# samanseifi/pyRMT

Measured on AMD Instinct MI355X. Metric: cell-updates/s (full RMT step) at N=4096; achieved HBM GB/s vs peak, higher is better.
Workload: dtype f64; 1 GPU; soft_disc_in_lid_driven N=4096 semilagrangian (configs 2/4 loop body); grid=4096, parallelism=single-gpu

## Files before the change

### pyrmt_amd/csrc/extrap.hip

```cpp
#include "extrap.hpp"
#include <cstring>
#include "exp_glibc.h"

namespace rmt {

constexpr int EXW = 8;
constexpr int EX_RING = 1024;
constexpr int EX_WIN = 81;
constexpr unsigned EX_DONE = 0x7fffffffu;
constexpr long EX_SPIN_LIMIT = 1L << 25;

__global__ void __launch_bounds__(256) k_ex_bits(const double *__restrict__ phi, int ny, int nx,
                                                 int W, int ML, u64 *__restrict__ kbits,
                                                 u64 *__restrict__ K,
                                                 unsigned char *__restrict__ rowcand,
                                                 int *__restrict__ jrange,
                                                 const double *__restrict__ X1,
                                                 const double *__restrict__ X2,
                                                 double *__restrict__ X1o,
                                                 double *__restrict__ X2o, int copy,
                                                 const u64 *__restrict__ kin) {
    const int j = blockIdx.y, i = blockIdx.x * 256 + threadIdx.x;
    const long c = (long)j * nx + i;
    const bool in = i < nx;
// ... 607 lines not shown
    const int ML = std::max(max_layers, 1), W = (nx + 63) / 64;
    const long plane = (long)ny * W;
    const long interior = (long)std::max(ny - 2, 0) * std::max(nx - 2, 0);
    const long maxt = std::max(64L, std::min((long)ML * interior, 4L * ML * (nx + ny) + 4096));
    char *p = (char *)base;
    size_t o = 0;
    auto take = [&](size_t n) { char *q = p ? p + o : nullptr; o += (n + 255) & ~(size_t)255; return q; };
    ExWs w{};
    w.kbits = (u64 *)take(plane * 8);
    w.cbits = (u64 *)take(plane * 8);
    w.Kold = (u64 *)take(plane * 8 * ML);
    w.rowcand = (unsigned char *)take(ny);
    w.jrange = (int *)take(64);
    w.status = w.jrange + 2;
    w.T = (u64 *)take(plane * 8 * ML);
    w.ACC = (u64 *)take(plane * 8 * ML);
    w.KN = (u64 *)take(plane * 8 * ML);
    w.rowcnt = (int *)take((size_t)ML * ny * 4);
    w.rowoff = (int *)take((size_t)ML * (ny + 1) * 4);
    w.wordoff = (int *)take(plane * 4 * ML);
    w.cbase = (int *)take((size_t)ML * ny * 4);
    w.tcell = (long long *)take(maxt * 8);
    w.recoff = (long long *)take(maxt * 8);
    w.rec_by_chain = (long long *)take(maxt * 8);
    w.chain_of = (int *)take(maxt * 4);
    w.dmark = (int *)take(maxt * 4);
    w.part = (unsigned char *)take(maxt);
    w.loc = (int *)take(maxt * 4);
    w.inv = (int *)take(maxt * 4);
    w.wnext = (int *)take(maxt * 4);
    w.gval = (double *)take(maxt * 16);
    w.rej = (int *)take((size_t)ML * EX_MAXREJ * 4);
    w.ctl = (int *)take(EXC_WORDS * 4);
    const long long cap = (1LL << 31) - 65536;
    w.slots = !bump && maxt * (long long)CH_MAXREC <= cap;
    w.arena_bytes = w.slots ? maxt * (long long)CH_MAXREC : std::min(maxt * 2560LL, cap);
    w.arena = take(w.arena_bytes);
    w.maxt = maxt;
    w.plane = plane;
    w.maxseg = maxt / PX_K + EX_MAXL + 2;
    if (px) {
        w.pns = (int *)take(maxt * 4);
        w.pnd = (int *)take(maxt * 4);
        w.pkey = (int *)take(maxt * PX_S * 4);
        w.pbeta = (double *)take(maxt * PX_S * 8);
        w.pval = (double2 *)take(maxt * 16);
        w.pc = (double2 *)take(maxt * 16);
        w.live = (unsigned char *)take(maxt);
        w.shdr = (int *)take(w.maxseg * PX_H * 4);
        w.sF = (int *)take(w.maxseg * PX_F * 4);
        w.sMT = (double *)take(w.maxseg * PX_F * PX_K * 8);
        w.sNT = (double *)take(w.maxseg * PX_K * PX_K * 8);
        w.sd = (double2 *)take(w.maxseg * PX_K * 16);
        w.spk = (double *)take(w.maxseg * PX_PB * 8);
    }
    if (bytes) *bytes = o;
    return w;
}

int extrap_none_rows(rmt_ctx *ctx, const u64 *kbits, int ny, int nx, double dx, double dy,
                     int jb, int je, int *ctl) {
    const double r = 4 * std::sqrt(dx * dx + dy * dy);
    if (je > jb)
        k_ex_none<<<grid1d(je - jb, 4), 256, 0, ctx->stream>>>(kbits, ny, nx, (nx + 63) / 64, dx,
                                                               dy, r * r, ctl, jb, je);
    RMT_LAUNCHED();
    return RMT_OK;
}

size_t extrap_workspace(int ny, int nx, int max_layers, bool px) {
    size_t b = 0;
    extrap_layout(nullptr, ny, nx, max_layers, &b, px);
    return b;
}

int extrap_geometry(rmt_ctx *ctx, const double *X1, const double *X2, const double *phi,
                    double dx, double dy, int max_layers, double *X1o, double *X2o,
                    const u64 *kin, const ExtrapCall &call) {
    const int ny = ctx->ny, nx = ctx->nx;
    const int W = (nx + 63) / 64;
    RMT_CHECK(max_layers > 0 && ny >= 3 && nx >= 3 && ny < (1 << 20) && nx < (1 << 30),
              RMT_EINVAL, "extrapolation grid size");
    const int force = g_ex_mode;
    const bool chain = force != 1 && extrap_chain_supported(ny, nx, max_layers);
    const bool par = chain && force == 0 && extrap_par_enabled();
    RMT_TRY(ensure_bytes(ctx, extrap_workspace(ny, nx, max_layers, par)));
    const ExWs ws = extrap_layout(ctx->bytes, ny, nx, max_layers, nullptr, par,
                                  ctx->opt.ex_arena_bump);
    ctx->ex_layers = max_layers;
    ctx->ex_chain = chain;
    ctx->ex_par = par;
    const int copy = (X1o != X1) || (X2o != X2);
    if (kin && !copy)
        k_ex_bits_w<<<grid1d((long)ny * W, 256), 256, 0, ctx->stream>>>(
            kin, ny, W, max_layers, ws.kbits, ws.Kold, ws.rowcand, ws.jrange);
    else
        k_ex_bits<<<dim3((nx + 255) / 256, ny), 256, 0, ctx->stream>>>(
            phi, ny, nx, W, max_layers, ws.kbits, ws.Kold, ws.rowcand, ws.jrange, X1, X2, X1o,
            X2o, copy, kin);
    RMT_HIP(hipMemsetAsync(ws.status, 0, 4 * sizeof(int), ctx->stream));
    if (chain) {
        RMT_HIP(hipMemsetAsync(ws.ctl, 0, EXC_WORDS * sizeof(int), ctx->stream));
        if (force == 2) {
            const int one = 1;
            RMT_HIP(hipMemcpyAsync(ws.ctl + EXC_FALLBACK, &one, sizeof(int),
                                   hipMemcpyHostToDevice, ctx->stream));
        }
        const double r = 4 * std::sqrt(dx * dx + dy * dy);
        int jb = 0, je = ny;
        if (call.none_rows[1] > call.none_rows[0]) {
            jb = std::max(0, call.none_rows[0]);
            je = std::min(ny, call.none_rows[1]);
        }
        if (call.none_wide && call.cand && je > jb) {
            int *cnt = call.cand + call.cand_cap;
            RMT_HIP(hipMemsetAsync(cnt, 0, sizeof(int), ctx->stream));
            int wb = 0, we = W;
            if (call.none_cols[1] > call.none_cols[0]) {
                wb = std::max(0, call.none_cols[0]);
                we = std::min(W, call.none_cols[1]);
            }
            k_ex_cand<<<grid1d((long)(je - jb) * (we - wb), 256), 256, 0, ctx->stream>>>(
                ws.kbits, ny, nx, W, jb, je, wb, we, call.cand, call.cand_cap, cnt);
            k_ex_none_list<<<1024, 256, 0, ctx->stream>>>(ws.kbits, ny, nx, W, dx, dy, r * r,
                                                           ws.ctl, jb, je, call.cand,
                                                           call.cand_cap, cnt);
        } else {
            k_ex_none<<<call.none_wide ? grid1d(std::max(je - jb, 1), 4)
                                          : std::min<unsigned>(grid1d(ny, 4), 64),
                        256, 0, ctx->stream>>>(
                ws.kbits, ny, nx, W, dx, dy, r * r, ws.ctl, jb, je);
        }
        k_ex_none_fin<<<1, 1, 0, ctx->stream>>>(ws.ctl);
        RMT_LAUNCHED();
        if (call.none_host && force == 0) {
            int any = 1;
            RMT_HIP(hipMemcpyAsync(&any, ws.ctl + EXC_ANY, sizeof(int), hipMemcpyDeviceToHost,
                                   ctx->stream));
            RMT_HIP(hipStreamSynchronize(ctx->stream));
            if (!any) { ctx->ex_noop_skip = true; return RMT_OK; }
        }
        if (par) {
            RMT_TRY(extrap_chain_prep_px(ctx, ws, dx, dy, max_layers));
            RMT_TRY(extrap_par_geometry(ctx, ws, dx, dy, max_layers));
        } else {
            RMT_TRY(extrap_chain_prep(ctx, ws, X1o, X2o, dx, dy, max_layers));
        }
    }
    const int *ctl = chain ? ws.ctl : nullptr;
    k_ex_dilate<<<grid1d((long)ny * W, 256), 256, 0, ctx->stream>>>(
        ws.kbits, ny, nx, W, max_layers, ws.cbits, ws.rowcand, ws.jrange, ctl);
    RMT_LAUNCHED();
    return RMT_OK;
}

int extrap_finish(rmt_ctx *ctx, double dx, double dy, int max_layers, double *X1o, double *X2o,
                  int *dev_status, const ExtrapCall &call) {
    const int ny = ctx->ny, nx = ctx->nx;
    const int W = (nx + 63) / 64;
    const bool par = ctx->ex_par;
    const ExWs ws = extrap_layout(ctx->bytes, ny, nx, max_layers, nullptr, par,
                                  ctx->opt.ex_arena_bump);
    const int force = g_ex_mode;
    if (ctx->ex_noop_skip) {
        ctx->ex_noop_skip = false;
        if (dev_status) RMT_HIP(hipMemsetAsync(dev_status, 0, 2 * sizeof(int), ctx->stream));
        if (call.chain_event) RMT_HIP(hipEventRecord(call.chain_event, ctx->stream));
        return RMT_OK;
    }
    const bool chain = ctx->ex_chain && !par;
    const int *ctl = ctx->ex_chain ? ws.ctl : nullptr;
    if (chain) RMT_TRY(extrap_chain_values(ctx, ws, X1o, X2o, dx, dy, max_layers, call));
    if (ctx->prof && !chain && !par) RMT_HIP(hipEventRecord(ctx->ev[2], ctx->stream));
    ExSweep A{X1o, X2o, ws.kbits, ws.cbits, ws.Kold, ws.rowcand, ws.jrange, ny, nx, W,
              max_layers, dx, dy, ws.status, ctl};
    const bool prof = ctx->opt.ex_profile != 0;
    const bool defer = chain && call.sweep_deferred && call.chain_event;
    RMT_CHECK(!defer || !dev_status, RMT_EINVAL,
              "extrap_finish: a deferred sweep leaves the status to the caller");
    if (defer) {
    } else if (!prof) {
        k_ex_sweep<false><<<1, EXW * 64, 0, ctx->stream>>>(A, nullptr);
        RMT_LAUNCHED();
    } else {
        long long *gp = nullptr, hp[EX_NPROF];
        int hs[2];
        RMT_HIP(hipMalloc(&gp, sizeof(hp)));
        RMT_HIP(hipMemsetAsync(gp, 0, sizeof(hp), ctx->stream));
        hipEvent_t e0, e1;
        RMT_HIP(hipEventCreate(&e0)); RMT_HIP(hipEventCreate(&e1));
        RMT_HIP(hipEventRecord(e0, ctx->stream));
        k_ex_sweep<true><<<1, EXW * 64, 0, ctx->stream>>>(A, gp);
        RMT_LAUNCHED();
        RMT_HIP(hipEventRecord(e1, ctx->stream));
        RMT_HIP(hipMemcpyAsync(hp, gp, sizeof(hp), hipMemcpyDeviceToHost, ctx->stream));
        RMT_HIP(hipMemcpyAsync(hs, ws.status, sizeof(hs), hipMemcpyDeviceToHost, ctx->stream));
        RMT_HIP(hipStreamSynchronize(ctx->stream));
        float ms = 0;
        RMT_HIP(hipEventElapsedTime(&ms, e0, e1));
        fprintf(stderr, "[ex-prof] %.3f ms fitted=%d rows=%lld | ticket+targets %.3g rowwait %.3g "
                "window %.3g wait %.3g load %.3g sum %.3g solve+store %.3g (Mclk, all waves)\n",
                ms, hs[0], hp[7], hp[0] / 1e6, hp[6] / 1e6, hp[1] / 1e6, hp[2] / 1e6,
                hp[3] / 1e6, hp[4] / 1e6, hp[5] / 1e6);
        (void)hipEventDestroy(e0); (void)hipEventDestroy(e1); (void)hipFree(gp);
    }
// ... 124 lines not shown
```

### pyrmt_amd/csrc/extrap.hpp

```cpp
#pragma once
#include "rmt_internal.hpp"

namespace rmt {

typedef unsigned long long u64;

constexpr int EX_MAXL = 8;
constexpr int CH_R = 2048;
#ifndef RMT_CH_W
#define RMT_CH_W 16
#endif
constexpr int CH_W = RMT_CH_W;
constexpr int CH_HDR = 24;
constexpr int CH_TVS = 88;
constexpr int CH_MAXREC = 8 * (CH_HDR + 6 * CH_TVS + 4 * 64);
constexpr int EX_MAXREJ = 4096;
constexpr int EX_DCAP = 8192;

constexpr int CH_MAXP = 8;
enum { EXC_FALLBACK = 0, EXC_ABORT = 1, EXC_FILLED = 2, EXC_ARENA = 4, EXC_REJ = 8,
       EXC_BASE = 8 + EX_MAXL, EXC_ANY = 8 + 2 * EX_MAXL, EXC_NOOP = EXC_ANY + 1,
       EXC_CMIN = EXC_ANY + 2, EXC_CMAX = EXC_ANY + 3, EXC_NPART = EXC_ANY + 4,
       EXC_WSTART = EXC_NPART + CH_MAXP + 1,
       EXC_NCOL = EXC_WSTART + CH_MAXP * CH_W,
       EXC_NLG = EXC_NCOL + 1,
       EXC_WORDS = EXC_NLG + 8 };
constexpr unsigned long long CH_GSENT = 0x7ff00000000bad01ull;
enum { EXA_CHAIN = 1, EXA_RELINK = 7, EXA_SWEEP = 8, EXA_PAR = 9 };
constexpr int EXA_TAG = 1 << 30;
__device__ __forceinline__ int exa_code(int kind, int part, int id) {
    return EXA_TAG | (kind << 26) | ((part & 15) << 22) | (id < 0 ? 0x3fffff : min(id, 0x3fffff));
}
__device__ __forceinline__ void exa_report(int *status, int code) {
    atomicCAS(status + 1, 0, code);
}
constexpr int PX_K = 64;
constexpr int PX_F = 64;
constexpr int PX_S = 81;
constexpr int PX_H = 8;
constexpr int PX_PB = 768;

struct ExWs {
    u64 *kbits, *cbits, *Kold;
    unsigned char *rowcand;
    int *jrange, *status;
    u64 *T, *ACC, *KN;
    int *rowcnt, *rowoff, *wordoff, *cbase;
    long long *tcell, *recoff, *rec_by_chain;
    int *chain_of, *dmark;
    unsigned char *part;
    int *loc, *inv;
    int *wnext;
    double *gval;
    int *rej;
    int *ctl;
    int *pns, *pnd;
    int *pkey;
    double *pbeta;
    double2 *pval, *pc;
    unsigned char *live;
    int *shdr, *sF;
    double *sMT, *sNT;
    double2 *sd;
    double *spk;
    long maxseg;
    char *arena;
    long long arena_bytes;
    int slots;
    long maxt;
    long plane;
};

ExWs extrap_layout(void *base, int ny, int nx, int max_layers, size_t *bytes, bool px = false,
                   bool bump = false);
int extrap_chain_prep(rmt_ctx *ctx, const ExWs &ws, const double *X1o, const double *X2o,
                      double dx, double dy, int ML);
int extrap_chain_values(rmt_ctx *ctx, const ExWs &ws, const double *X1o, const double *X2o,
                        double dx, double dy, int ML, const ExtrapCall &call = {});
int extrap_chain_run(rmt_ctx *ctx, const ExWs &ws, const double *X1o, const double *X2o, int ML,
                     const ExtrapCall &call = {});
bool extrap_chain_supported(int ny, int nx, int ML);
int extrap_chain_prep_px(rmt_ctx *ctx, const ExWs &ws, double dx, double dy, int ML);
int extrap_par_geometry(rmt_ctx *ctx, const ExWs &ws, double dx, double dy, int ML);
int extrap_par_values(rmt_ctx *ctx, const ExWs &ws, double *X1o, double *X2o, int ML);

}
```

### pyrmt_amd/csrc/extrap_chain.hip

```cpp
#include "extrap.hpp"
#include "exp_glibc.h"
#include <algorithm>
#include <cstdio>
#include <cstdlib>
#include <vector>

namespace rmt {

constexpr int EXS = 82;
constexpr long long CH_CRIT = 1LL << 16;

__device__ __forceinline__ u64 ld_l2(const u64 *p) {
    return __hip_atomic_load(p, __ATOMIC_RELAXED, __HIP_MEMORY_SCOPE_AGENT);
}
__device__ __forceinline__ int wave_incl_scan(int v, int lane) {
#pragma unroll
    for (int d = 1; d < 64; d <<= 1) {
        const int t = __shfl_up(v, d);
        if (lane >= d) v += t;
    }
    return v;
}
__device__ __forceinline__ u64 rl64(u64 v, int l) {
    const unsigned lo = __builtin_amdgcn_readlane((unsigned)v, l);
    const unsigned hi = __builtin_amdgcn_readlane((unsigned)(v >> 32), l);
    return ((u64)hi << 32) | lo;
}
__device__ __forceinline__ double rlf(double v, int l) {
    return __longlong_as_double((long long)rl64((u64)__double_as_longlong(v), l));
}
__device__ __forceinline__ int ex_id(const ExWs &ws, int ny, int Ls, int jj, long o, u64 bit) {
    return ws.ctl[EXC_BASE + Ls] + ws.rowoff[(long)Ls * (ny + 1) + jj] +
           ws.wordoff[(long)Ls * ws.plane + o] + __popcll(ws.T[(long)Ls * ws.plane + o] & (bit - 1));
}

__global__ void __launch_bounds__(256) k_tg_rows(ExWs ws, int ny, int nx, int W, int L) {
    const int lane = threadIdx.x & 63, j = blockIdx.x * 4 + (threadIdx.x >> 6);
    if (j >= ny) return;
    const long plane = ws.plane;
    const u64 *Kpp = L >= 2 ? ws.KN + (long)(L - 2) * plane : ws.kbits;
    const u64 *Ap = L >= 1 ? ws.ACC + (long)(L - 1) * plane : nullptr;
    auto K = [&](int jj, int w) -> u64 {
        if (jj < 0 || jj >= ny || w < 0 || w >= W) return 0;
// ... 138 lines not shown
    __builtin_amdgcn_fence(__ATOMIC_SEQ_CST, "wavefront");
    double acc = 0.0;
    if (lane < 6) {
        const double2 *t2 = (const double2 *)(tb + lane * EXS);
        double2 t[40];
#pragma unroll
        for (int q2 = 0; q2 < 40; ++q2) t[q2] = t2[q2];
        const double last = tb[lane * EXS + 80];
#pragma unroll
        for (int q2 = 0; q2 < 40; ++q2) { acc += t[q2].x; acc += t[q2].y; }
        acc += last;
    }
    __builtin_amdgcn_wave_barrier();
    __builtin_amdgcn_fence(__ATOMIC_SEQ_CST, "wavefront");
    const double A00 = rlf(acc, 0), A01 = rlf(acc, 1), A02 = rlf(acc, 2);
    const double A11 = rlf(acc, 3), A12 = rlf(acc, 4), A22 = rlf(acc, 5);
    const double M[9] = {A00, A01, A02, A01, A11, A12, A02, A12, A22};
    const double det = (M[0] * (M[4] * M[8] - M[5] * M[7])
                      - M[1] * (M[3] * M[8] - M[5] * M[6])
                      + M[2] * (M[3] * M[7] - M[4] * M[6]));
    const bool accept = count >= 3 && fabs(det) > 1e-10;
    if (!accept) {
        if (lane == 0) ws.recoff[id] = -1;
        return false;
    }
    if (A.norec) return true;
    const u64 lt = (1ull << lane) - 1;
    const u64 tl = il & ~((qf >= 64) ? ~0ull : ((1ull << qf) - 1));
    const u64 th = ih & ~((qf >= 64) ? ((1ull << (qf - 64)) - 1) : 0ull);
    const int n = __popcll(tl) + __popcll(th), npad = (n + 7) & ~7;
    const int nd = __popcll(dl) + __popcll(dh);
    const long long bytes = ((8LL * (CH_HDR + 4 * nd + 6 * npad)) + 63) & ~63LL;
    unsigned long long off = 0;
    if (nd > 64) {
        if (lane == 0) { ws.ctl[EXC_FALLBACK] = 1; ws.recoff[id] = -1; }
        return true;
    }
    if (ws.slots) {
        off = (unsigned long long)id * CH_MAXREC;
    } else {
        if (lane == 0) {
            off = atomicAdd((unsigned long long *)(ws.ctl + EXC_ARENA), (unsigned long long)bytes);
            if ((long long)(off + bytes) > ws.arena_bytes) ws.ctl[EXC_FALLBACK] = 1;
        }
        off = rl64(off, 0);
    }
    if ((long long)(off + bytes) > ws.arena_bytes) {
        if (lane == 0) ws.recoff[id] = -1;
        return true;
    }
    double *rec = (double *)(ws.arena + off);
    double *dyn = rec + CH_HDR;
    double *tv = dyn + 4 * nd;
#pragma unroll
    for (int h = 0; h < 2; ++h) {
        const bool term = h ? ((th >> lane) & 1) && lane < 17 : (tl >> lane) & 1;
        if (!term) continue;
        const int k = h ? __popcll(tl) + __popcll(th & lt) : __popcll(tl & lt);
        const double wa0 = w[h] * 1.0, wa1 = w[h] * xi[h], wa2 = w[h] * yi[h];
        if (!st[h]) {
            const int dk = h ? __popcll(dl) + __popcll(dh & lt) : __popcll(dl & lt);
            dyn[4 * dk] = __longlong_as_double(((long long)src[h] << 32) | (unsigned)k);
            dyn[4 * dk + 1] = wa0; dyn[4 * dk + 2] = wa1; dyn[4 * dk + 3] = wa2;
        }
    }
    if (lane < 6 * (npad - n)) tv[(lane / (npad - n)) * npad + n + lane % (npad - n)] = 0.0;
    if (lane == 0) {
// ... 107 lines not shown
            const double2 *t2 = (const double2 *)(T + lane * EXS);
            double2 t[40];
#pragma unroll
            for (int q2 = 0; q2 < 40; ++q2) t[q2] = t2[q2];
            const double last = T[lane * EXS + 80];
#pragma unroll
            for (int q2 = 0; q2 < 40; ++q2) { acc += t[q2].x; acc += t[q2].y; }
            acc += last;
        }
        __builtin_amdgcn_wave_barrier();
        __builtin_amdgcn_fence(__ATOMIC_SEQ_CST, "wavefront");
        double *rec = (double *)(ws.arena + ((r & 0xffffffffLL) << 6));
        const long long meta = __double_as_longlong(rec[1]);
        const int npad = (int)(meta & 0xffffffff), nd = (int)((meta >> 32) & 0x7fffffff);
        double *tv = rec + CH_HDR + 4 * nd;
        const u64 il = __ballot(inc[0]), ih = __ballot(inc[1] && lane < 17);
        const u64 lt = (1ull << lane) - 1;
        const u64 tl = il & ~((qf >= 64) ? ~0ull : ((1ull << qf) - 1));
        const u64 th = ih & ~((qf >= 64) ? ((1ull << (qf - 64)) - 1) : 0ull);
#pragma unroll
        for (int h = 0; h < 2; ++h) {
            const bool term = h ? ((th >> lane) & 1) && lane < 17 : (tl >> lane) & 1;
            if (!term || !st[h]) continue;
            const int k = h ? __popcll(tl) + __popcll(th & lt) : __popcll(tl & lt);
            const double wa0 = w[h] * 1.0, wa1 = w[h] * xi[h], wa2 = w[h] * yi[h];
            tv[0 * npad + k] = wa0 * b1[h]; tv[1 * npad + k] = wa1 * b1[h];
            tv[2 * npad + k] = wa2 * b1[h]; tv[3 * npad + k] = wa0 * b2[h];
            tv[4 * npad + k] = wa1 * b2[h]; tv[5 * npad + k] = wa2 * b2[h];
        }
        if (lane < 6) rec[17 + lane] = acc;
    }
}

constexpr int FIXW = 8;

__device__ void ex_add_dependents(const ExGeoArgs &A, int id, int *dlist, int *dn) {
    const ExWs &ws = A.ws;
    const long c = ws.tcell[id];
    const int j = (int)(c / A.nx), i = (int)(c % A.nx);
    const u64 *T = ws.T + (long)A.L * ws.plane;
    for (int jj = j; jj <= min(A.ny - 1, j + 4); ++jj)
        for (int ii = max(0, i - 4); ii <= min(A.nx - 1, i + 4); ++ii) {
            if (jj == j && ii <= i) continue;
            const long o = (long)jj * A.W + (ii >> 6);
            const u64 bit = 1ull << (ii & 63);
            if (!(T[o] & bit)) continue;
            const int d = ex_id(ws, A.ny, A.L, jj, o, bit);
            if (atomicExch(ws.dmark + d, 1) == 1) continue;
            const int p = atomicAdd(dn, 1);
            if (p < EX_DCAP) dlist[p] = d;
        }
}

__global__ void __launch_bounds__(FIXW * 64) k_ex_fix(ExGeoArgs A) {
    __shared__ u64 tab[256];
    __shared__ __attribute__((aligned(16))) double tb[FIXW][6 * EXS];
    __shared__ int dlist[EX_DCAP];
    __shared__ unsigned char dres[EX_DCAP];
    __shared__ int dn, nflip;
    const ExWs &ws = A.ws;
    const int nrej = ws.ctl[EXC_REJ + A.L];
    if (nrej == 0 || ws.ctl[EXC_FALLBACK]) return;
    for (int s = threadIdx.x; s < 256; s += blockDim.x) tab[s] = kExpTab[s];
    if (threadIdx.x == 0) dn = 0;
    __syncthreads();
    for (int r = threadIdx.x; r < min(nrej, EX_MAXREJ); r += blockDim.x)
// ... 61 lines not shown
    }
}

__global__ void __launch_bounds__(1024) k_ex_split(ExWs ws, int nx, int ML, int ncol, int nlg) {
    __shared__ int smin[1024], smax[1024];
    const int t = threadIdx.x, total = ws.ctl[EXC_BASE + ML];
    int mn = 0x7fffffff, mx = -1;
    for (int id = t; id < total; id += 1024) {
        const int i = (int)(ws.tcell[id] % nx);
        mn = min(mn, i); mx = max(mx, i);
    }
    smin[t] = mn; smax[t] = mx;
    __syncthreads();
    for (int w = 512; w > 0; w >>= 1) {
        if (t < w) { smin[t] = min(smin[t], smin[t + w]); smax[t] = max(smax[t], smax[t + w]); }
        __syncthreads();
    }
    if (t == 0) {
        ws.ctl[EXC_CMIN] = smin[0];
        ws.ctl[EXC_CMAX] = smax[0] >= smin[0] ? smax[0] - smin[0] + 1 : 1;
        ws.ctl[EXC_NCOL] = ncol;
        ws.ctl[EXC_NLG] = nlg;
        ws.ctl[EXC_NPART + CH_MAXP] = ncol * nlg;
    }
}
__device__ __forceinline__ int ch_col_of(const int *ctl, int i) {
    const int np = ctl[EXC_NCOL];
    if (np <= 1) return 0;
    const long q = (long)(i - ctl[EXC_CMIN]) * np / ctl[EXC_CMAX];
    return (int)min((long)np - 1, max(0L, q));
}

__global__ void __launch_bounds__(256) k_ex_chainidx(ExWs ws, int ny, int nx, int ML,
                                                     int *status) {
    if (ws.ctl[EXC_FALLBACK]) return;
    const int id = blockIdx.x * 256 + threadIdx.x, total = ws.ctl[EXC_BASE + ML];
    bool acc = false;
    if (id < total) {
        int L = ML - 1;
        while (L > 0 && id < ws.ctl[EXC_BASE + L]) --L;
        const int j = (int)(ws.tcell[id] / nx);
        const int x = ws.cbase[(long)L * ny + j] +
                      (id - ws.ctl[EXC_BASE + L] - ws.rowoff[(long)L * (ny + 1) + j]);
        ws.chain_of[id] = x;
        const int nlg = ws.ctl[EXC_NLG];
        ws.part[x] = (unsigned char)(ch_col_of(ws.ctl, (int)(ws.tcell[id] % nx)) * nlg +
                                     L * nlg / ML);
        const long long r = ws.recoff[id];
        ws.rec_by_chain[x] = r;
        acc = r >= 0;
    }
    const u64 b = __ballot(acc);
    if ((threadIdx.x & 63) == 0 && b) atomicAdd(status, __popcll(b));
}

__global__ void __launch_bounds__(1024) k_ex_local(ExWs ws, int ML) {
    __shared__ int sc[CH_MAXP][1024];
    if (ws.ctl[EXC_FALLBACK]) return;
    const int t = threadIdx.x, total = ws.ctl[EXC_BASE + ML], per = (total + 1023) / 1024;
    const int a = min(total, t * per), b = min(total, a + per);
    int cnt[CH_MAXP];
#pragma unroll
    for (int p = 0; p < CH_MAXP; ++p) cnt[p] = 0;
    for (int x = a; x < b; ++x) {
        const int px = ws.part[x];
#pragma unroll
        for (int p = 0; p < CH_MAXP; ++p) cnt[p] += px == p;
    }
#pragma unroll
    for (int p = 0; p < CH_MAXP; ++p) sc[p][t] = cnt[p];
    __syncthreads();
    for (int d = 1; d < 1024; d <<= 1) {
        int v[CH_MAXP];
#pragma unroll
        for (int p = 0; p < CH_MAXP; ++p) v[p] = t >= d ? sc[p][t - d] : 0;
        __syncthreads();
#pragma unroll
        for (int p = 0; p < CH_MAXP; ++p) sc[p][t] += v[p];
        __syncthreads();
    }
    int base[CH_MAXP], run[CH_MAXP];
    int acc = 0;
#pragma unroll
    for (int p = 0; p < CH_MAXP; ++p) {
        base[p] = acc; acc += sc[p][1023];
        run[p] = sc[p][t] - cnt[p];
// ... 449 lines not shown
        const long long nx = __double_as_longlong(B[23]);
        const int x2 = __builtin_amdgcn_readfirstlane((int)(nx >> 32));
        const unsigned r2 = (unsigned)__builtin_amdgcn_readfirstlane((int)(nx & 0xffffffff));
        if (x2 <= x) { ok = false; break; }
        if (x2 < total) CH_LOAD(r2);
        CH_STAMP(6);
        const bool fit_ok = ch_fit<PROF>(x, lane, B, val, tag, cur, wm, o, c, pr, tl,
                                         C.ws.gval, base + x, C.trace, base);
        if (!fit_ok) { ok = false; break; }
        x = x2; r = r2;
    }
    if constexpr (PROF)
        if (lane == 0)
            for (int k = 0; k < 12; ++k) atomicAdd((unsigned long long *)&gprof[k], pr[k]);
    if (ok && c >= 0 && (lane == 0 || lane == CH_XL2)) (lane == 0 ? X1e : X2e)[c] = o;
    __hip_atomic_store(&cur[wv], 0x7fffffff, __ATOMIC_RELAXED, __HIP_MEMORY_SCOPE_WORKGROUP);
    if (!ok && lane == 0) {
        C.ws.ctl[EXC_ABORT] = 1;
        exa_report(C.status, exa_code(EXA_CHAIN, part, x));
    }
}
static int chain_parts(const rmt_ctx *ctx, int ML, int *ncol, int *nlg) {
    *ncol = std::min(CH_MAXP, std::max(1, ctx->opt.ch_cols));
    int g = ctx->opt.ch_lgroups > 0 ? ctx->opt.ch_lgroups : ML;
    *nlg = std::max(1, std::min({g, ML, CH_MAXP / *ncol}));
    return *ncol * *nlg;
}

bool extrap_chain_supported(int ny, int nx, int ML) {
    return ML >= 1 && ML <= EX_MAXL && ny >= 3 && nx >= 3;
}

int extrap_chain_prep(rmt_ctx *ctx, const ExWs &ws, const double *X1o, const double *X2o,
                      double dx, double dy, int ML) {
    const int ny = ctx->ny, nx = ctx->nx, W = (nx + 63) / 64;
    hipStream_t st = ctx->stream;
    const unsigned rows = grid1d(ny, 4);
    double r = 4 * std::sqrt(dx * dx + dy * dy);
    ExGeoArgs A{ws, X1o, X2o, ny, nx, W, 0, dx, dy, r * r, 0};
    const unsigned gblocks = (unsigned)std::min<long>(4096, std::max<long>(1, ws.maxt / 4));
    for (int L = 0; L < ML; ++L) {
        A.L = L;
        k_tg_rows<<<rows, 256, 0, st>>>(ws, ny, nx, W, L);
        k_tg_scan<<<1, 1024, 0, st>>>(ws, ny, L);
        k_tg_emit<<<rows, 256, 0, st>>>(ws, ny, nx, W, L);
        k_ex_geom<<<gblocks, 256, 0, st>>>(A);
        k_ex_fix<<<1, FIXW * 64, 0, st>>>(A);
        RMT_LAUNCHED();
    }
    int ncol, nlg;
    const int nparts = chain_parts(ctx, ML, &ncol, &nlg);
    k_ex_order<<<1, 1024, 0, st>>>(ws, ny, ML);
    k_ex_split<<<1, 1024, 0, st>>>(ws, nx, ML, ncol, nlg);
    const unsigned idb = grid1d(ws.maxt, 256);
    k_ex_chainidx<<<idb, 256, 0, st>>>(ws, ny, nx, ML, ws.status);
    k_ex_local<<<1, 1024, 0, st>>>(ws, ML);
    k_ex_runs<<<nparts, 1024, 0, st>>>(ws);
    k_ex_relink<<<std::min<unsigned>(grid1d(ws.maxt, 4), 2048), 256, 0, st>>>(ws, ML);
    RMT_LAUNCHED();
    return RMT_OK;
}

int extrap_chain_prep_px(rmt_ctx *ctx, const ExWs &ws, double dx, double dy, int ML) {
    const int ny = ctx->ny, nx = ctx->nx, W = (nx + 63) / 64;
    hipStream_t st = ctx->stream;
    const unsigned rows = grid1d(ny, 4);
    double r = 4 * std::sqrt(dx * dx + dy * dy);
    ExGeoArgs A{ws, nullptr, nullptr, ny, nx, W, 0, dx, dy, r * r, 1};
    const unsigned gblocks = (unsigned)std::min<long>(4096, std::max<long>(1, ws.maxt / 4));
    for (int L = 0; L < ML; ++L) {
        A.L = L;
        k_tg_rows<<<rows, 256, 0, st>>>(ws, ny, nx, W, L);
        k_tg_scan<<<1, 1024, 0, st>>>(ws, ny, L);
        k_tg_emit<<<rows, 256, 0, st>>>(ws, ny, nx, W, L);
        k_ex_geom<<<gblocks, 256, 0, st>>>(A);
        k_ex_fix<<<1, FIXW * 64, 0, st>>>(A);
        RMT_LAUNCHED();
    }
    return RMT_OK;
}

int extrap_chain_values(rmt_ctx *ctx, const ExWs &ws, const double *X1o, const double *X2o,
                        double dx, double dy, int ML, const ExtrapCall &call) {
    const int ny = ctx->ny, nx = ctx->nx, W = (nx + 63) / 64;
    const double r = 4 * std::sqrt(dx * dx + dy * dy);
    ExGeoArgs A{ws, X1o, X2o, ny, nx, W, 0, dx, dy, r * r, 0};
    const unsigned gblocks = (unsigned)std::min<long>(4096, std::max<long>(1, ws.maxt / 4));
    RMT_HIP(launch_done(ctx, k_ex_vals, dim3(gblocks), dim3(256), 0, ctx->stream,
                        call.event_with_values ? call.chain_event : nullptr, A, ML));
    return RMT_OK;
}

int extrap_chain_run(rmt_ctx *ctx, const ExWs &ws, const double *X1o, const double *X2o,
                     int ML, const ExtrapCall &call) {
    hipStream_t st = ctx->stream;
    int ncol, nlg;
    const int nparts = chain_parts(ctx, ML, &ncol, &nlg);
    if (ctx->prof) RMT_HIP(hipEventRecord(ctx->ev[2], st));
    if (call.chain_event && !call.event_with_values)
        RMT_HIP(hipEventRecord(call.chain_event, st));
    ChainArgs C{ws, (double *)X1o, (double *)X2o, ML, ws.status, nullptr};
    if (!ctx->opt.ex_profile) {
        k_ex_chain<false><<<nparts, CH_W * 64, 0, st>>>(C, nullptr);
        RMT_LAUNCHED();
    } else {
        long long *gp = nullptr, hp[12];
        RMT_HIP(hipMalloc(&gp, sizeof(hp)));
        RMT_HIP(hipMemsetAsync(gp, 0, sizeof(hp), st));
        hipEvent_t e0, e1;
        RMT_HIP(hipEventCreate(&e0)); RMT_HIP(hipEventCreate(&e1));
        static const char *tpath = getenv("RMT_EX_TRACE");
        static bool traced = false;
        long long *dtr = nullptr;
        if (tpath && !traced) {
            RMT_HIP(hipMalloc(&dtr, 6 * sizeof(long long) * ws.maxt));
            RMT_HIP(hipMemsetAsync(dtr, 0, 6 * sizeof(long long) * ws.maxt, st));
            C.trace = dtr;
        }
        RMT_HIP(hipEventRecord(e0, st));
        k_ex_chain<true><<<nparts, CH_W * 64, 0, st>>>(C, gp);
        RMT_LAUNCHED();
        RMT_HIP(hipEventRecord(e1, st));
// ... 31 lines not shown
```

### pyrmt_amd/csrc/ops.hip

```cpp
#include "rmt_internal.hpp"
#include <algorithm>
#include <cstdio>
#include <cstring>
#include <mutex>
#include <vector>

namespace rmt {
static thread_local std::string g_err;
void set_error(const std::string &m) { g_err = m; }
static const struct { const char *name, *env; int rmt_opts::*f; } kOpts[] = {
    {"ext_events", "RMT_EXT_EVENTS", &rmt_opts::ext_events},
    {"ex_arena_bump", nullptr, &rmt_opts::ex_arena_bump},
    {"ex_profile", "RMT_EX_PROFILE", &rmt_opts::ex_profile},
    {"fix_all", "RMT_FIX_ALL", &rmt_opts::fix_all},
    {"dct_rocfft", "RMT_DCT_ROCFFT", &rmt_opts::dct_rocfft},
    {"transpose2", "RMT_TRANSPOSE2", &rmt_opts::transpose2},
    {"sim_hiprio", "RMT_SIM_HIPRIO", &rmt_opts::sim_hiprio},
    {"sim_sync", "RMT_SIM_SYNC", &rmt_opts::sim_sync},
    {"early_geometry", "RMT_EARLY_GEOMETRY", &rmt_opts::early_geometry},
    {"early_transpose", "RMT_EARLY_TRANSPOSE", &rmt_opts::early_transpose},
    {"fused_fluid", "RMT_FUSED_FLUID", &rmt_opts::fused_fluid},
    {"no_overlap", "RMT_NO_OVERLAP", &rmt_opts::no_overlap},
    {"side_tail", "RMT_SIDE_TAIL", &rmt_opts::side_tail},
    {"par_overlap", "RMT_PAR_OVERLAP", &rmt_opts::par_overlap},
    {"fused_fixprep", "RMT_FUSED_FIXPREP", &rmt_opts::fused_fixprep},
    {"merged_join", "RMT_MERGED_JOIN", &rmt_opts::merged_join},
    {"test_delay_side", "RMT_TEST_DELAY_SIDE", &rmt_opts::test_delay_side},
    {"test_delay_main", "RMT_TEST_DELAY_MAIN", &rmt_opts::test_delay_main},
    {"test_delay_geo", "RMT_TEST_DELAY_GEO", &rmt_opts::test_delay_geo},
    {"test_nowait_drop", "RMT_TEST_NOWAIT_DROP", &rmt_opts::test_nowait_drop},
    {"chain_cols", "RMT_CH_PARTS", &rmt_opts::ch_cols},
    {"chain_layer_groups", "RMT_CH_LAYERS", &rmt_opts::ch_lgroups},
    {"edge_slots", "RMT_EDGE_SLOTS_USED", &rmt_opts::edge_slots},
    {"edge_stream", "RMT_EDGE_STREAM", &rmt_opts::edge_stream},
    {"sl_phi", "RMT_SL_PHI", &rmt_opts::sl_phi},
    {"mac_boxes", "RMT_MAC_BOXES", &rmt_opts::mac_boxes},
    {"skip_marked_rows", "RMT_SKIP_MARKED_ROWS", &rmt_opts::skip_marked_rows},
    {"tail_stream", "RMT_TAIL_STREAM", &rmt_opts::tail_stream},
    {"diag_first", "RMT_DIAG_FIRST", &rmt_opts::diag_first},
    {"mac_noop_host", "RMT_MAC_NOOP_HOST", &rmt_opts::mac_noop_host},
    {"mac_face_sl", "RMT_MAC_FACE_SL", &rmt_opts::mac_face_sl},
    {"mac_m2_bound", "RMT_MAC_M2_BOUND", &rmt_opts::mac_m2_bound},
    {"diag_seg", "RMT_DIAG_SEG", &rmt_opts::diag_seg},
    {"sl_zero_flags", "RMT_SL_ZERO_FLAGS", &rmt_opts::sl_zero_flags},
    {"dct_sym", "RMT_DCT_SYM", &rmt_opts::dct_sym},
};
// ... 1058 lines not shown
```

### pyrmt_amd/csrc/rmt_internal.hpp

```cpp
#pragma once
#include <hip/hip_runtime.h>
#include <hip/hip_ext.h>
#include <rocfft/rocfft.h>
#include <algorithm>
#include <cmath>
#include <cstdint>
#include <string>
#include "../../include/rmt.h"
#include "divk.hpp"

namespace rmt {

constexpr int LIST_BLOCKS = 1024;
extern int g_list_blocks;
inline unsigned list_grid(long max_tiles) {
    return (unsigned)std::max(1L, std::min<long>(max_tiles, g_list_blocks));
}

__host__ __device__ __forceinline__ double nanmax(double a, double b) {
    return (a != a || b != b) ? (a + b) : (a > b ? a : b);
}


void set_error(const std::string &msg);
// ... 6 lines not shown
        }                                                                               \
    } while (0)
#define RMT_LAUNCHED()                                                                  \
    do {                                                                                \
        hipError_t e_ = hipGetLastError();                                              \
        if (e_ != hipSuccess) {                                                         \
            ::rmt::set_error(std::string(__FILE__) + ":" + std::to_string(__LINE__) +   \
                             " launch: " + hipGetErrorString(e_));                      \
            return RMT_EDEVICE;                                                         \
        }                                                                               \
    } while (0)
#define RMT_CHECK(cond, code, msg)                                                      \
    do {                                                                                \
        if (!(cond)) { ::rmt::set_error(msg); return (code); }                          \
    } while (0)
#define RMT_UPLOAD(dst, src, bytes)                                                     \
    do {                                                                                \
        RMT_HIP(hipMemcpy((dst), (src), (bytes), hipMemcpyHostToDevice));               \
        RMT_HIP(hipDeviceSynchronize());                                                \
    } while (0)
#define RMT_TRY(expr)                                                                   \
    do { int s_ = (expr); if (s_ != RMT_OK) return s_; } while (0)

struct DctPlan;
struct Dct2Plan;
struct PerPlan;

}

struct rmt_opts {
    int ext_events = 1;
    int ex_arena_bump = 0;
    int ex_profile = 0;
    int fix_all = 0;
    int dct_rocfft = 0;
    int transpose2 = 1;
    int sim_hiprio = 1;
    int sim_sync = 0;
    int early_geometry = 1;
    int early_transpose = 1;
    int fused_fluid = 1;
    int no_overlap = 0;
    int side_tail = 1;
    int par_overlap = 1;
    int fused_fixprep = 1;
    int merged_join = 1;
    int test_delay_side = 0;
    int test_delay_main = 0;
    int test_delay_geo = 0;
    int test_nowait_drop = 0;
    int ch_cols = 2;
    int ch_lgroups = 0;
    int edge_slots = 64;
    int edge_stream = 1;
    int sl_phi = 1;
    int mac_boxes = 1;
    int skip_marked_rows = 1;
    int tail_stream = 1;
    int diag_first = 0;
    int mac_noop_host = 1;
    int mac_face_sl = 1;
    int mac_m2_bound = 1;
    int diag_seg = 1;
    int dct_sym = 1;
    int sl_zero_flags = 1;
};

#define RMT_EDGE_PRIOS 2
#ifndef RMT_EDGE_SLOTS
#define RMT_EDGE_SLOTS 64
#endif
struct rmt_ctx {
    int ny = 0, nx = 0, device = 0;
    hipStream_t stream = nullptr;
    double *scratch = nullptr;
    size_t scratch_bytes = 0;
    double *red = nullptr;
    double *rsum = nullptr;
    int rsum_len = 0;
    unsigned char *bytes = nullptr;
    size_t bytes_len = 0;
    unsigned long bytes_gen = 0;
    rmt::DctPlan *dct = nullptr;
    rmt::Dct2Plan *dct2 = nullptr;
    rmt::PerPlan *per = nullptr;
    bool prof = false;
    hipEvent_t ev[4] = {nullptr, nullptr, nullptr, nullptr};
    int ex_layers = 0;
    bool ex_chain = false;
    bool ex_par = false;
    bool ex_noop_skip = false;
    struct EdgeTiles { int *list = nullptr; int n = 0; long key[6] = {}; };
    EdgeTiles edge[RMT_EDGE_SLOTS];
    int edge_next = 0;
    hipStream_t edge_sts[RMT_EDGE_PRIOS] = {};
    int edge_prios[RMT_EDGE_PRIOS] = {};
    hipEvent_t edge_ev[9] = {};
    void *imex[2] = {nullptr, nullptr};
    rmt_opts opt;
};
static_assert(sizeof(((rmt_ctx *)nullptr)->edge) / sizeof(rmt_ctx::EdgeTiles) == RMT_EDGE_SLOTS, "edge slots");

namespace rmt {

struct StreamScope {
    rmt_ctx *ctx;
    hipStream_t prev;
    StreamScope(rmt_ctx *c, hipStream_t s) : ctx(c), prev(c->stream) { c->stream = s; }
    ~StreamScope() { ctx->stream = prev; }
    StreamScope(const StreamScope &) = delete;
    StreamScope &operator=(const StreamScope &) = delete;
};

int ensure_scratch(rmt_ctx *ctx, size_t bytes);
int ensure_bytes(rmt_ctx *ctx, size_t bytes);
inline unsigned grid1d(long n, int block) { return (unsigned)((n + block - 1) / block); }

template <typename... Formals, typename... Actuals>
inline hipError_t launch_done(const rmt_ctx *ctx, void (*k)(Formals...), dim3 g, dim3 b,
                              uint32_t lds, hipStream_t s, hipEvent_t done, Actuals... a) {
    if (done && ctx->opt.ext_events) {
        hipExtLaunchKernelGGL(k, g, b, lds, s, nullptr, done, 0, a...);
        return hipGetLastError();
// ... 526 lines not shown
```

Baseline: 5.671 billion cell-updates/s.

## Precompute chain extrapolation stencil plan during prep and use compact values kernel

Adds a plan kernel that runs during chain prep, before the value stage. For each accepted chain cell it records the stencil masks, the layer, the first-dependent index and the record metadata into a compact plan buffer. The value stage then reads this plan and no longer recomputes the bitplane lookups, which takes bitmask work off the path between geometry and values. It adds plan-index allocation in the chain-index kernel, a larger workspace, and a new fallback when a record exceeds a size bound.

```diff
diff --git a/pyrmt_amd/csrc/extrap.hip b/pyrmt_amd/csrc/extrap.hip
--- a/pyrmt_amd/csrc/extrap.hip
+++ b/pyrmt_amd/csrc/extrap.hip
@@ -663,6 +663,8 @@
     w.gval = (double *)take(maxt * 16);
     w.rej = (int *)take((size_t)ML * EX_MAXREJ * 4);
     w.ctl = (int *)take(EXC_WORDS * 4);
+    w.plan = (u64 *)take(maxt * 64);
+    w.planidx = (int *)take(maxt * 4);
     const long long cap = (1LL << 31) - 65536;
     w.slots = !bump && maxt * (long long)CH_MAXREC <= cap;
     w.arena_bytes = w.slots ? maxt * (long long)CH_MAXREC : std::min(maxt * 2560LL, cap);
@@ -721,6 +723,7 @@
     ctx->ex_layers = max_layers;
     ctx->ex_chain = chain;
     ctx->ex_par = par;
+    ctx->ex_plan = chain && !par && ctx->opt.ex_plan != 0;
     const int copy = (X1o != X1) || (X2o != X2);
     if (kin && !copy)
         k_ex_bits_w<<<grid1d((long)ny * W, 256), 256, 0, ctx->stream>>>(
@@ -775,7 +778,7 @@
             RMT_TRY(extrap_chain_prep_px(ctx, ws, dx, dy, max_layers));
             RMT_TRY(extrap_par_geometry(ctx, ws, dx, dy, max_layers));
         } else {
-            RMT_TRY(extrap_chain_prep(ctx, ws, X1o, X2o, dx, dy, max_layers));
+            RMT_TRY(extrap_chain_prep(ctx, ws, X1o, X2o, dx, dy, max_layers, ctx->ex_plan));
         }
     }
     const int *ctl = chain ? ws.ctl : nullptr;
@@ -801,7 +804,8 @@
     }
     const bool chain = ctx->ex_chain && !par;
     const int *ctl = ctx->ex_chain ? ws.ctl : nullptr;
-    if (chain) RMT_TRY(extrap_chain_values(ctx, ws, X1o, X2o, dx, dy, max_layers, call));
+    if (chain)
+        RMT_TRY(extrap_chain_values(ctx, ws, X1o, X2o, dx, dy, max_layers, ctx->ex_plan, call));
     if (ctx->prof && !chain && !par) RMT_HIP(hipEventRecord(ctx->ev[2], ctx->stream));
     ExSweep A{X1o, X2o, ws.kbits, ws.cbits, ws.Kold, ws.rowcand, ws.jrange, ny, nx, W,
               max_layers, dx, dy, ws.status, ctl};
diff --git a/pyrmt_amd/csrc/extrap.hpp b/pyrmt_amd/csrc/extrap.hpp
--- a/pyrmt_amd/csrc/extrap.hpp
+++ b/pyrmt_amd/csrc/extrap.hpp
@@ -24,6 +24,7 @@
        EXC_WSTART = EXC_NPART + CH_MAXP + 1,
        EXC_NCOL = EXC_WSTART + CH_MAXP * CH_W,
        EXC_NLG = EXC_NCOL + 1,
+       EXC_NPLAN = EXC_NLG + 1,
        EXC_WORDS = EXC_NLG + 8 };
 constexpr unsigned long long CH_GSENT = 0x7ff00000000bad01ull;
 enum { EXA_CHAIN = 1, EXA_RELINK = 7, EXA_SWEEP = 8, EXA_PAR = 9 };
@@ -53,6 +54,8 @@
     int *wnext;
     double *gval;
     int *rej;
+    u64 *plan;
+    int *planidx;
     int *ctl;
     int *pns, *pnd;
     int *pkey;
@@ -74,9 +77,9 @@
 ExWs extrap_layout(void *base, int ny, int nx, int max_layers, size_t *bytes, bool px = false,
                    bool bump = false);
 int extrap_chain_prep(rmt_ctx *ctx, const ExWs &ws, const double *X1o, const double *X2o,
-                      double dx, double dy, int ML);
+                      double dx, double dy, int ML, bool plan);
 int extrap_chain_values(rmt_ctx *ctx, const ExWs &ws, const double *X1o, const double *X2o,
-                        double dx, double dy, int ML, const ExtrapCall &call = {});
+                        double dx, double dy, int ML, bool plan, const ExtrapCall &call = {});
 int extrap_chain_run(rmt_ctx *ctx, const ExWs &ws, const double *X1o, const double *X2o, int ML,
                      const ExtrapCall &call = {});
 bool extrap_chain_supported(int ny, int nx, int ML);
diff --git a/pyrmt_amd/csrc/extrap_chain.hip b/pyrmt_amd/csrc/extrap_chain.hip
--- a/pyrmt_amd/csrc/extrap_chain.hip
+++ b/pyrmt_amd/csrc/extrap_chain.hip
@@ -9,6 +9,7 @@
 
 constexpr int EXS = 82;
 constexpr long long CH_CRIT = 1LL << 16;
+constexpr int CH_LOADP = 5;
 
 __device__ __forceinline__ u64 ld_l2(const u64 *p) {
     return __hip_atomic_load(p, __ATOMIC_RELAXED, __HIP_MEMORY_SCOPE_AGENT);
@@ -213,7 +214,7 @@
     const int nd = __popcll(dl) + __popcll(dh);
     const long long bytes = ((8LL * (CH_HDR + 4 * nd + 6 * npad)) + 63) & ~63LL;
     unsigned long long off = 0;
-    if (nd > 64) {
+    if (nd > 64 || bytes > CH_LOADP * 64 * 16) {
         if (lane == 0) { ws.ctl[EXC_FALLBACK] = 1; ws.recoff[id] = -1; }
         return true;
     }
@@ -387,6 +388,144 @@
     }
 }
 
+__global__ void __launch_bounds__(256) k_ex_plan(ExGeoArgs A, int ML) {
+    const ExWs &ws = A.ws;
+    if (ws.ctl[EXC_FALLBACK]) return;
+    const int lane = threadIdx.x & 63, wv = threadIdx.x >> 6;
+    const int total = ws.ctl[EXC_BASE + ML];
+    const int W = A.W, nx = A.nx, ny = A.ny;
+    const long plane = ws.plane;
+    for (int id = blockIdx.x * 4 + wv; id < total; id += gridDim.x * 4) {
+        const long long r = ws.recoff[id];
+        if (r < 0) continue;
+        int L = ML - 1;
+        while (L > 0 && id < ws.ctl[EXC_BASE + L]) --L;
+        const long c = ws.tcell[id];
+        const int j = (int)(c / nx), i = (int)(c % nx);
+        const u64 *Kst = L == 0 ? ws.kbits : ws.KN + (long)(L - 1) * plane;
+        const u64 *SL = ws.ACC + (long)L * plane;
+        const double x0 = A.dx * i, y0 = A.dy * j;
+        bool inc[2], st[2];
+#pragma unroll
+        for (int h = 0; h < 2; ++h) {
+            const int q = lane + 64 * h, jj = j - 4 + q / 9, ii = i - 4 + q % 9;
+            inc[h] = false; st[h] = false;
+            const double xi = A.dx * ii, yi = A.dy * jj;
+            if (q < 81 && jj >= 0 && jj < ny && ii >= 0 && ii < nx) {
+                const double ax = xi - x0, ay = yi - y0, d2 = ax * ax + ay * ay;
+                if (d2 <= A.r2) {
+                    const long o = (long)jj * W + (ii >> 6);
+                    const u64 bit = 1ull << (ii & 63);
+                    const bool ks = (Kst[o] & bit) != 0;
+                    bool sl = false;
+                    if (!ks && (jj < j || (jj == j && ii < i))) sl = (SL[o] & bit) != 0;
+                    inc[h] = ks || sl;
+                    if (inc[h]) st[h] = (ws.kbits[o] & bit) != 0;
+                }
+            }
+        }
+        const u64 il = __ballot(inc[0]), ih = __ballot(inc[1] && lane < 17);
+        const u64 sl = __ballot(st[0]), sh = __ballot(st[1] && lane < 17);
+        const u64 dl = il & ~sl, dh = ih & ~sh;
+        const int qf = dl ? __builtin_ctzll(dl) : (dh ? 64 + __builtin_ctzll(dh) : 81);
+        const double *rec = (const double *)(ws.arena + ((r & 0xffffffffLL) << 6));
+        const long long meta = __double_as_longlong(rec[1]);
+        const u64 npad = (u64)(meta & 0xffffffff), nd = (u64)((meta >> 32) & 0x7fffffff);
+        const int e = ws.planidx[id];
+        if (e < 0 || e >= ws.maxt) continue;
+        u64 v = 0;
+        if (lane == 0) v = (u64)c | ((u64)L << 48) | ((u64)qf << 56);
+        if (lane == 1) v = il;
+        if (lane == 2) v = ih | (sh << 32);
+        if (lane == 3) v = sl;
+        if (lane == 4) v = (u64)(r & 0xffffffffLL) | (npad << 32) | (nd << 48);
+        if (lane < 8) ws.plan[8L * e + lane] = v;
+    }
+}
+
+__global__ void __launch_bounds__(256) k_ex_vals_plan(ExGeoArgs A) {
+    __shared__ __attribute__((aligned(16))) double tb[4][6 * EXS];
+    const ExWs &ws = A.ws;
+    if (ws.ctl[EXC_FALLBACK]) return;
+    const int n = (int)min((long)ws.ctl[EXC_NPLAN], ws.maxt);
+    const int lane = threadIdx.x & 63, wv = threadIdx.x >> 6;
+    const int nx = A.nx;
+    double *T = tb[wv];
+    for (int e = blockIdx.x * 4 + wv; e < n; e += gridDim.x * 4) {
+        const u64 pw = ws.plan[8L * e + (lane & 7)];
+        const u64 p0 = rl64(pw, 0), il = rl64(pw, 1), p2 = rl64(pw, 2), sl = rl64(pw, 3);
+        const u64 p4 = rl64(pw, 4);
+        const u64 ih = p2 & 0xffffffffull, sh = p2 >> 32;
+        const long c = (long)(p0 & ((1ull << 48) - 1));
+        const int qf = (int)(p0 >> 56);
+        const int j = (int)(c / nx), i = (int)(c % nx);
+        const double x0 = A.dx * i, y0 = A.dy * j;
+        bool st[2];
+        double w[2], xi[2], yi[2], b1[2], b2[2];
+#pragma unroll
+        for (int h = 0; h < 2; ++h) {
+            const int q = lane + 64 * h, jj = j - 4 + q / 9, ii = i - 4 + q % 9;
+            st[h] = h ? lane < 17 && ((sh >> lane) & 1) : (sl >> lane) & 1;
+            w[h] = 0.0; b1[h] = 0.0; b2[h] = 0.0;
+            xi[h] = A.dx * ii; yi[h] = A.dy * jj;
+            if (st[h]) {
+                const long cc = (long)jj * nx + ii;
+                b1[h] = A.X1[cc]; b2[h] = A.X2[cc];
+                const double ax = xi[h] - x0, ay = yi[h] - y0, d2 = ax * ax + ay * ay;
+                w[h] = exp_glibc(-d2 / A.r2);
+            }
+        }
+        const int np2 = min(40, (qf + 1) >> 1);
+#pragma unroll
+        for (int h = 0; h < 2; ++h) {
+            const int q = lane + 64 * h;
+            if (q >= 81) break;
+            const double wa0 = w[h] * 1.0, wa1 = w[h] * xi[h], wa2 = w[h] * yi[h];
+            const bool pre = st[h] && q < qf;
+            T[0 * EXS + q] = pre ? wa0 * b1[h] : 0.0;
+            T[1 * EXS + q] = pre ? wa1 * b1[h] : 0.0;
+            T[2 * EXS + q] = pre ? wa2 * b1[h] : 0.0;
+            T[3 * EXS + q] = pre ? wa0 * b2[h] : 0.0;
+            T[4 * EXS + q] = pre ? wa1 * b2[h] : 0.0;
+            T[5 * EXS + q] = pre ? wa2 * b2[h] : 0.0;
+        }
+        __builtin_amdgcn_wave_barrier();
+        __builtin_amdgcn_fence(__ATOMIC_SEQ_CST, "wavefront");
+        double acc = 0.0;
+        if (lane < 6) {
+            const double2 *t2 = (const double2 *)(T + lane * EXS);
+            for (int q0 = 0; q0 < np2; q0 += 4) {
+                double2 t[4];
+#pragma unroll
+                for (int k = 0; k < 4; ++k) t[k] = t2[min(q0 + k, 39)];
+#pragma unroll
+                for (int k = 0; k < 4; ++k)
+                    if (q0 + k < np2) { acc += t[k].x; acc += t[k].y; }
+            }
+            if (qf > 80) acc += T[lane * EXS + 80];
+        }
+        __builtin_amdgcn_wave_barrier();
+        __builtin_amdgcn_fence(__ATOMIC_SEQ_CST, "wavefront");
+        double *rec = (double *)(ws.arena + ((p4 & 0xffffffffull) << 6));
+        const int npad = (int)((p4 >> 32) & 0xffff), nd = (int)(p4 >> 48);
+        double *tv = rec + CH_HDR + 4 * nd;
+        const u64 lt = (1ull << lane) - 1;
+        const u64 tl = il & ~((qf >= 64) ? ~0ull : ((1ull << qf) - 1));
+        const u64 th = ih & ~((qf >= 64) ? ((1ull << (qf - 64)) - 1) : 0ull);
+#pragma unroll
+        for (int h = 0; h < 2; ++h) {
+            const bool term = h ? ((th >> lane) & 1) && lane < 17 : (tl >> lane) & 1;
+            if (!term || !st[h]) continue;
+            const int k = h ? __popcll(tl) + __popcll(th & lt) : __popcll(tl & lt);
+            const double wa0 = w[h] * 1.0, wa1 = w[h] * xi[h], wa2 = w[h] * yi[h];
+            tv[0 * npad + k] = wa0 * b1[h]; tv[1 * npad + k] = wa1 * b1[h];
+            tv[2 * npad + k] = wa2 * b1[h]; tv[3 * npad + k] = wa0 * b2[h];
+            tv[4 * npad + k] = wa1 * b2[h]; tv[5 * npad + k] = wa2 * b2[h];
+        }
+        if (lane < 6) rec[17 + lane] = acc;
+    }
+}
+
 constexpr int FIXW = 8;
 
 __device__ void ex_add_dependents(const ExGeoArgs &A, int id, int *dlist, int *dn) {
@@ -514,7 +653,7 @@
 }
 
 __global__ void __launch_bounds__(256) k_ex_chainidx(ExWs ws, int ny, int nx, int ML,
-                                                     int *status) {
+                                                     int *status, int plan) {
     if (ws.ctl[EXC_FALLBACK]) return;
     const int id = blockIdx.x * 256 + threadIdx.x, total = ws.ctl[EXC_BASE + ML];
     bool acc = false;
@@ -534,6 +673,13 @@
     }
     const u64 b = __ballot(acc);
     if ((threadIdx.x & 63) == 0 && b) atomicAdd(status, __popcll(b));
+    if (plan && b) {
+        const int lane = threadIdx.x & 63;
+        int e0 = 0;
+        if (lane == 0) e0 = atomicAdd(ws.ctl + EXC_NPLAN, __popcll(b));
+        e0 = __shfl(e0, 0);
+        if (acc) ws.planidx[id] = e0 + __popcll(b & ((1ull << lane) - 1));
+    }
 }
 
 __global__ void __launch_bounds__(1024) k_ex_local(ExWs ws, int ML) {
@@ -1049,7 +1195,7 @@
 }
 
 int extrap_chain_prep(rmt_ctx *ctx, const ExWs &ws, const double *X1o, const double *X2o,
-                      double dx, double dy, int ML) {
+                      double dx, double dy, int ML, bool plan) {
     const int ny = ctx->ny, nx = ctx->nx, W = (nx + 63) / 64;
     hipStream_t st = ctx->stream;
     const unsigned rows = grid1d(ny, 4);
@@ -1070,10 +1216,11 @@
     k_ex_order<<<1, 1024, 0, st>>>(ws, ny, ML);
     k_ex_split<<<1, 1024, 0, st>>>(ws, nx, ML, ncol, nlg);
     const unsigned idb = grid1d(ws.maxt, 256);
-    k_ex_chainidx<<<idb, 256, 0, st>>>(ws, ny, nx, ML, ws.status);
+    k_ex_chainidx<<<idb, 256, 0, st>>>(ws, ny, nx, ML, ws.status, plan);
     k_ex_local<<<1, 1024, 0, st>>>(ws, ML);
     k_ex_runs<<<nparts, 1024, 0, st>>>(ws);
     k_ex_relink<<<std::min<unsigned>(grid1d(ws.maxt, 4), 2048), 256, 0, st>>>(ws, ML);
+    if (plan) k_ex_plan<<<gblocks, 256, 0, st>>>(A, ML);
     RMT_LAUNCHED();
     return RMT_OK;
 }
@@ -1098,13 +1245,18 @@
 }
 
 int extrap_chain_values(rmt_ctx *ctx, const ExWs &ws, const double *X1o, const double *X2o,
-                        double dx, double dy, int ML, const ExtrapCall &call) {
+                        double dx, double dy, int ML, bool plan, const ExtrapCall &call) {
     const int ny = ctx->ny, nx = ctx->nx, W = (nx + 63) / 64;
     const double r = 4 * std::sqrt(dx * dx + dy * dy);
     ExGeoArgs A{ws, X1o, X2o, ny, nx, W, 0, dx, dy, r * r, 0};
+    hipEvent_t ev = call.event_with_values ? call.chain_event : nullptr;
+    if (plan) {
+        RMT_HIP(launch_done(ctx, k_ex_vals_plan, dim3(grid1d(ws.maxt, 4)), dim3(256), 0,
+                            ctx->stream, ev, A));
+        return RMT_OK;
+    }
     const unsigned gblocks = (unsigned)std::min<long>(4096, std::max<long>(1, ws.maxt / 4));
-    RMT_HIP(launch_done(ctx, k_ex_vals, dim3(gblocks), dim3(256), 0, ctx->stream,
-                        call.event_with_values ? call.chain_event : nullptr, A, ML));
+    RMT_HIP(launch_done(ctx, k_ex_vals, dim3(gblocks), dim3(256), 0, ctx->stream, ev, A, ML));
     return RMT_OK;
 }
 
diff --git a/pyrmt_amd/csrc/ops.hip b/pyrmt_amd/csrc/ops.hip
--- a/pyrmt_amd/csrc/ops.hip
+++ b/pyrmt_amd/csrc/ops.hip
@@ -12,6 +12,7 @@
     {"ext_events", "RMT_EXT_EVENTS", &rmt_opts::ext_events},
     {"ex_arena_bump", nullptr, &rmt_opts::ex_arena_bump},
     {"ex_profile", "RMT_EX_PROFILE", &rmt_opts::ex_profile},
+    {"ex_plan", "RMT_EX_PLAN", &rmt_opts::ex_plan},
     {"fix_all", "RMT_FIX_ALL", &rmt_opts::fix_all},
     {"dct_rocfft", "RMT_DCT_ROCFFT", &rmt_opts::dct_rocfft},
     {"transpose2", "RMT_TRANSPOSE2", &rmt_opts::transpose2},
diff --git a/pyrmt_amd/csrc/rmt_internal.hpp b/pyrmt_amd/csrc/rmt_internal.hpp
--- a/pyrmt_amd/csrc/rmt_internal.hpp
+++ b/pyrmt_amd/csrc/rmt_internal.hpp
@@ -62,6 +62,7 @@
     int ext_events = 1;
     int ex_arena_bump = 0;
     int ex_profile = 0;
+    int ex_plan = 1;
     int fix_all = 0;
     int dct_rocfft = 0;
     int transpose2 = 1;
@@ -119,6 +120,7 @@
     int ex_layers = 0;
     bool ex_chain = false;
     bool ex_par = false;
+    bool ex_plan = false;
     bool ex_noop_skip = false;
     struct EdgeTiles { int *list = nullptr; int n = 0; long key[6] = {}; };
     EdgeTiles edge[RMT_EDGE_SLOTS];
```

New measurement: 5.666 billion cell-updates/s. No clear change (-0.1%).
